# CliqueOfficial/zk-dcap-verifier

Measured on AMD Instinct MI355X. Metric: proofs/hour sgx_dcap_verifier k=19 (create_proof on the GPU: commitments, lookups, grand products, NTTs, evaluate_h, evaluations, SHPLONK, host transcript; witness synthesis excluded), higher is better.
Workload: dtype u32x8 (256-bit Montgomery integers)

## Files before the change

### zk-dcap-verifier_amd/csrc/capi.hip

```cpp
#include <string.h>
#include <new>
#include <system_error>
#include "quotient.h"

namespace zk {
int ntt_set_lds_attr();
int quotient_set_lds_attr();
int domain_lagrange_to_coeff(zk_ctx* ctx, void* d_a, uint32_t k);
int domain_coeff_to_lagrange(zk_ctx* ctx, void* d_a, uint32_t k);
int domain_lagrange_to_coeff_batch(zk_ctx* ctx, void* const* cols, size_t count, uint32_t k);
int domain_coeff_to_extended_batch(zk_ctx* ctx, const void* const* coeffs, void* const* outs, size_t count, uint32_t k, uint32_t ek);
int ntt_dev_batch(zk_ctx* ctx, void* const* h_cols, const void* const* h_srcs, size_t count, uint32_t log_n, const u256& omega, const NttFuse* fuse);
int domain_coeff_to_extended(zk_ctx* ctx, const void* d_coeff, uint32_t k, uint32_t ek, void* d_out);
int domain_extended_to_coeff(zk_ctx* ctx, void* d_a, uint32_t k, uint32_t ek);
int domain_divide_by_vanishing(zk_ctx* ctx, void* d_a, uint32_t k, uint32_t ek);
int fr_vec_op(zk_ctx* ctx, int op, const void* a, const void* b, void* out, size_t n, const u256* scalar);
int permutation_product(zk_ctx* ctx, const void* const* values, const void* const* sigmas, size_t count, uint32_t k, const void* beta, const void* gamma,
                        const void* delta_start, const void* z_init, const void* blinding, uint32_t bf, void* d_z, void* h_last_z);
int lookup_product(zk_ctx* ctx, const void* cin, const void* ctab, const void* pin, const void* ptab, uint32_t k, const void* beta, const void* gamma,
                   const void* blinding, uint32_t bf, void* d_z);
int permutation_product_circuits(zk_ctx* ctx, const void* const* values, const void* const* sigmas, size_t m, size_t n_circuits, uint32_t chunk_len, uint32_t k,
                                 const void* beta, const void* gamma, const void* blinding, uint32_t bf, void* const* d_zs);
int lookup_product_batch(zk_ctx* ctx, const void* const* cols4, size_t count, uint32_t k, const void* beta, const void* gamma, const void* blinding,
                         uint32_t bf, void* const* d_zs);
// ... 136 lines not shown
    std::unique_ptr<zk_ctx> ctx(new zk_ctx());
    ctx->device = device_id;
    if (hipStreamCreateWithFlags(&ctx->stream, hipStreamNonBlocking) != hipSuccess) return ZK_ERR_HIP;
    msm_set_lds_attr();
    ntt_set_lds_attr();
    quotient_set_lds_attr();
    *out = ctx.release();
    return ZK_OK;
} ZK_ABI_CATCH(nullptr)

}
zk_ctx* zk_internal_helper_ctx(zk_ctx* ctx) {
    if (!ctx) return nullptr;
    zk_ctx* h;
    {
        LOCK;
        h = ctx->helper;
    }
    if (!h) {
        zk_ctx* made = nullptr;
        if (zk_ctx_create(ctx->device, &made) != ZK_OK) return nullptr;
#ifndef ZK_EMU
        {
            int lane_prio;
            { LOCK; lane_prio = ctx->tune.prover_lane_priority; }
            int least = 0, greatest = 0;
            hipStream_t s = nullptr;
            if (lane_prio && hipDeviceGetStreamPriorityRange(&least, &greatest) == hipSuccess && least != greatest &&
                hipStreamCreateWithPriority(&s, hipStreamNonBlocking, lane_prio == 1 ? least : greatest) == hipSuccess) {
                (void)hipStreamDestroy(made->stream);
                made->stream = s;
            }
        }
#endif
        {
            LOCK;
            if (!ctx->helper) { ctx->helper = made; made = nullptr; }
            h = ctx->helper;
        }
        if (made) zk_ctx_destroy(made);
    }
    zk::Tune t;
    bool timing;
    {
        LOCK;
        t = ctx->tune; timing = ctx->timing;
    }
    std::lock_guard<std::mutex> lk(h->mu);
    h->tune = t;
    h->timing = timing;
    return h;
}
static void release_workspaces(zk_ctx* ctx) {
    zk::DevBuf* bufs[] = {&ctx->ws_scalars, &ctx->ws_sorted, &ctx->ws_mid, &ctx->ws_small, &ctx->ws_sub0, &ctx->ws_sub1, &ctx->ws_cls0,
                          &ctx->ws_cls1, &ctx->ws_tmp, &ctx->ws_ntt, &ctx->ws_ntt_in, &ctx->ws_pts, &ctx->ws_runs, &ctx->ws_quot, &ctx->ws_quot_state};
    for (auto* b : bufs) b->release();
}
void zk_internal_trim_helper(zk_ctx* ctx) {
    if (!ctx) return;
    zk_ctx* h;
    { LOCK; h = ctx->helper; }
    if (!h) return;
    std::lock_guard<std::mutex> lk(h->mu);
    (void)hipSetDevice(h->device);
    (void)hipStreamSynchronize(h->stream);
    release_workspaces(h);
    release_twiddles(h);
}
extern "C" {
void zk_ctx_destroy(zk_ctx* ctx) ZK_ABI_TRY {
    if (!ctx) return;
    zk_ctx* helper;
    { LOCK; helper = ctx->helper; ctx->helper = nullptr; }
    if (helper) zk_ctx_destroy(helper);
    zk_internal_plonk_ctx_destroyed(ctx);
    (void)zk_plonk_trim(ctx);
    {
        LOCK;
        (void)hipSetDevice(ctx->device);
        (void)hipStreamSynchronize(ctx->stream);
        ctx->bases.clear();
        drop_pending_timers(ctx);
        release_twiddles(ctx);
        release_pks(ctx);
        release_mock_sessions(ctx);
        release_programs(ctx);
        release_gtab(ctx);
        release_workspaces(ctx);
        (void)hipStreamDestroy(ctx->stream);
    }
    delete ctx;
} ZK_ABI_CATCH_VOID(ctx)

const char* zk_last_error(zk_ctx* ctx) ZK_ABI_TRY { return ctx ? ctx->err : "null context"; } ZK_ABI_CATCH_VALUE(ctx, "zkmi355: internal error")

static int* tune_slot(zk_ctx* ctx, const char* key) {
    zk::Tune& t = ctx->tune;
    struct { const char* k; int* v; } tab[] = {
        {"msm_c", &t.msm_c}, {"msm_sort_wgs", &t.msm_sort_wgs}, {"msm_sort_threads", &t.msm_sort_threads}, {"msm_sort_batch_wgs", &t.msm_sort_batch_wgs}, {"msm_bsort_threads", &t.msm_bsort_threads}, {"msm_bsort_chunk", &t.msm_bsort_chunk}, {"msm_wide_bins_log", &t.msm_wide_bins_log}, {"msm_part_threads", &t.msm_part_threads}, {"msm_part_pairs", &t.msm_part_pairs}, {"msm_two_level_sort", &t.msm_two_level_sort},
        {"msm_target_threads", &t.msm_target_threads}, {"msm_min_chunk", &t.msm_min_chunk}, {"msm_max_chunk", &t.msm_max_chunk},
        {"msm_max_chunk_wide", &t.msm_max_chunk_wide}, {"msm_merge_fanin", &t.msm_merge_fanin}, {"msm_tree_fanin", &t.msm_tree_fanin}, {"msm_block", &t.msm_block}, {"msm_runs", &t.msm_runs}, {"prover_side_lane", &t.prover_side_lane}, {"prover_lane_priority", &t.prover_lane_priority},
        {"ntt_tile_log", &t.ntt_tile_log}, {"ntt_threads", &t.ntt_threads}, {"ntt_max_radix_log", &t.ntt_max_radix_log}, {"ntt_plan", &t.ntt_plan}, {"ntt_full_twiddle_max_log", &t.ntt_full_twiddle_max_log}, {"ntt_coset_table", &t.ntt_coset_table}, {"ntt_col_major", &t.ntt_col_major},
        {"vec_block", &t.vec_block}, {"quot_threads", &t.quot_threads},
        {"ntt_quarter_input", &t.ntt_quarter_input}, {"ntt_fuse_scale", &t.ntt_fuse_scale}, {"quot_piece_cosets", &t.quot_piece_cosets}, {"quot_factor_horner", &t.quot_factor_horner}, {"quot_degree_split", &t.quot_degree_split}, {"quot_group_factors", &t.quot_group_factors}, {"ntt_ws_limit_mb", &t.ntt_ws_limit_mb}, 
        {"quot_jit", &t.quot_jit}, {"quot_jit_group", &t.quot_jit_group}, {"quot_jit_waves", &t.quot_jit_waves}, {"quot_remat_ops", &t.quot_remat_ops}, {"quot_remat_distance", &t.quot_remat_distance}, {"keygen_wgs", &t.keygen_wgs}, {"mock_edge_wgs", &t.mock_edge_wgs}};
    for (auto& e : tab) if (!strcmp(e.k, key)) return e.v;
    return nullptr;
// ... 330 lines not shown
```

### zk-dcap-verifier_amd/csrc/ctx.h

```cpp
#pragma once
#include <stdarg.h>
#include <string.h>
#include <stdio.h>
#include <list>
#include <map>
#include <memory>
#include <mutex>
#include <string>
#include <vector>
#include "ec.cuh"
#include "../../include/zkmi355.h"
#include "abi_guard.h"

namespace zk {

struct Tune {
    int msm_c = 0;
    int msm_sort_wgs = 256;
    int msm_sort_threads = 1024;
    int msm_bsort_threads = 1024;
    int msm_bsort_chunk = 8192;
    int msm_part_threads = 1024, msm_part_pairs = 16384;
    int msm_wide_bins_log = 9;
    int msm_two_level_sort = 0;
// ... 58 lines not shown
    void reset() { if (p) (void)hipFree(p); p = nullptr; }
};

struct TableMem {
    void* p = nullptr;
    int device = 0;
    ~TableMem() { if (p) { (void)hipSetDevice(device); (void)hipFree(p); } }
};
struct BaseTable {
    void* d_table = nullptr;
    size_t n = 0;
    int c = 0, W = 0;
    std::shared_ptr<TableMem> mem;
    void* d_runs_table = nullptr;
    std::shared_ptr<TableMem> runs_mem;
};

struct TwiddleSet {
    uint32_t log_n = 0;
    u256 omega;
    void* d_lo = nullptr;
    void* d_hi = nullptr;
    uint32_t lo_bits = 0;
    void* d_stage[3] = {nullptr, nullptr, nullptr};
    void* d_stage_sh[3] = {nullptr, nullptr, nullptr};
    void* d_stage29[3] = {nullptr, nullptr, nullptr};
    void* d_full[3] = {nullptr, nullptr, nullptr};
    uint32_t radix_log[3] = {0, 0, 0};
    int passes = 0;
    bool scale_fused = false;
    u256 fused_scale;
    uint64_t stamp = 0;
};

struct QuotProgram;
struct MockSession;

}

struct zk_ctx {
    int device = 0;
    std::mutex mu;
    char err[640] = {0};
    hipStream_t stream = nullptr;
    zk::Tune tune;
    uint64_t next_handle = 1;
    std::map<uint64_t, zk::BaseTable> bases;
    std::list<zk::TwiddleSet> twiddles;
    uint64_t twiddle_clock = 0;
    std::map<uint64_t, void*> coset_tables;
    std::map<uint64_t, std::shared_ptr<zk::QuotProgram>> programs;
    std::map<uint64_t, std::shared_ptr<zk::MockSession>> mock_sessions;
    std::map<uint64_t, std::vector<uint32_t>> lookup_tie_hint;
    zk::DevBuf ws_scalars, ws_sorted, ws_mid, ws_small, ws_sub0, ws_sub1, ws_cls0, ws_cls1, ws_tmp, ws_ntt, ws_ntt_in, ws_pts, ws_runs, ws_quot, ws_quot_state;
    bool timing = false;
    std::map<std::string, double> last_ms;
    struct PendingTimer { const char* label; hipEvent_t a, b; };
    std::vector<PendingTimer> pending_timers;
    zk_ctx* helper = nullptr;

    int fail(int code, const char* fmt, ...) {
        char buf[sizeof err];
        va_list ap;
        va_start(ap, fmt);
        vsnprintf(buf, sizeof buf, fmt, ap);
        va_end(ap);
        memcpy(err, buf, sizeof err);
        return code;
    }
};

#define ZK_HIP(call)                                                                          \
    do {                                                                                      \
        hipError_t e__ = (call);                                                              \
        if (e__ != hipSuccess)                                                                \
            return ctx->fail(ZK_ERR_HIP, "%s failed: %s (%s:%d)", #call, hipGetErrorString(e__), __FILE__, __LINE__); \
    } while (0)
#define ZK_CHECK_LAUNCH() ZK_HIP(hipGetLastError())

namespace zk {
inline void resolve_pending_timers(zk_ctx* ctx);
struct EvTimer {
    zk_ctx* ctx; const char* label; hipEvent_t a = nullptr, b = nullptr; bool on;
    EvTimer(zk_ctx* c, const char* l) : ctx(c), label(l), on(c->timing) {
        if (on) { (void)hipEventCreate(&a); (void)hipEventCreate(&b); (void)hipEventRecord(a, ctx->stream); }
    }
    void stop() { if (on) (void)hipEventRecord(b, ctx->stream); }
    void resolve() {
        if (!on) return;
        (void)hipEventSynchronize(b);
        float ms = 0; (void)hipEventElapsedTime(&ms, a, b);
        on = false;
        (void)hipEventDestroy(a); (void)hipEventDestroy(b);
        ctx->last_ms[label] += ms; ctx->last_ms[std::string(label) + "#n"] += 1.0;
    }
    void defer() {
        if (!on) return;
        if (ctx->pending_timers.size() >= 4096) resolve_pending_timers(ctx);
        ctx->pending_timers.push_back({label, a, b});
        on = false;
    }
    ~EvTimer() { if (on) { (void)hipEventDestroy(a); (void)hipEventDestroy(b); } }
    EvTimer(const EvTimer&) = delete;
    EvTimer& operator=(const EvTimer&) = delete;
};
inline void resolve_pending_timers(zk_ctx* ctx) {
    std::vector<zk_ctx::PendingTimer> list;
// ... 40 lines not shown
```

### zk-dcap-verifier_amd/csrc/msm.hip

```cpp
#include "ctx.h"
#include <algorithm>
#include <math.h>

namespace zk {

template <class F>
ZK_HD void for_each_digit(u256 s, int c, int W, F&& f) {
    const uint32_t mask = (1u << c) - 1u, half = 1u << (c - 1);
    uint32_t carry = 0;
    for (int j = 0; j < W; j++) {
        uint32_t d = (s.v[0] & mask) + carry;
#pragma unroll
        for (int i = 0; i < 7; i++) s.v[i] = (s.v[i] >> c) | (s.v[i + 1] << (32 - c));
        s.v[7] >>= c;
        if (d > half) {
            carry = 1;
            uint32_t m = (1u << c) - d;
            if (m) f(j, m, true);
        } else {
            carry = 0;
            if (d) f(j, d, false);
        }
    }
}
// ... 24 lines not shown
    uint32_t carry = 0;
#pragma unroll
    for (int j = 0; j < 16; j++) {
        const uint32_t d = ((s.v[j >> 1] >> (16 * (j & 1))) & 0xffffu) + carry;
        if (d > 0x8000u) {
            carry = 1;
            const uint32_t m = 0x10000u - d;
            if (m) f(j, m, true);
        } else {
            carry = 0;
            if (d) f(j, d, false);
        }
    }
}
template <int J = 0, class F>
ZK_HD void for_each_digit16_static(const u256& s, F&& f, uint32_t carry = 0) {
    if constexpr (J < 16) {
        const uint32_t d = ((s.v[J >> 1] >> (16 * (J & 1))) & 0xffffu) + carry;
        uint32_t cy = 0;
        if (d > 0x8000u) {
            cy = 1;
            const uint32_t m = 0x10000u - d;
            if (m) f(WinIdx<J>{}, m, true);
        } else if (d) f(WinIdx<J>{}, d, false);
        for_each_digit16_static<J + 1>(s, f, cy);
    }
}

ZK_HD uint32_t find_segment(const uint32_t* arr, uint32_t B, uint32_t j) {
    uint32_t lo = 0, hi = B;
    while (hi - lo > 1) {
        uint32_t mid = (lo + hi) >> 1;
        if (arr[mid] <= j) lo = mid; else hi = mid;
    }
    return lo;
}

ZK_HD uint32_t ceil_div(uint32_t a, uint32_t b) { return (a + b - 1) / b; }

constexpr int MSM_MAX_LEVELS = 12;
struct MsmPlan {
    uint32_t n, n_table, B, L, M, Mlog, R, nb;
    int c, W;
    const void* const* scalars;
    const void* table;
    const void* const* col_tables;
    uint32_t* small;
    uint32_t small_stride, o_off, o_cursor, o_suboff, o_info, o_tiles, o_fulloff, o_remorder, o_remhist, o_remstart, o_remcursor;
    uint32_t* sorted;
    uint64_t sorted_stride;
    uint32_t low_bits, nbin, pch, bch, o_bintot, o_bincur, o_binbase, o_chunkbase;
    uint32_t* mid_ref;
    uint16_t* mid_low;
    void* sub[2];
    uint64_t sub_stride[2];
    void* cls[2];
    uint32_t lo_bits;
};
ZK_HD uint32_t* plan_small(const MsmPlan& p, uint32_t col) { return p.small + (size_t)col * p.small_stride; }
ZK_HD const uint32_t* plan_suboff(const MsmPlan& p, uint32_t col, uint32_t level) { return plan_small(p, col) + p.o_suboff + (size_t)level * (p.B + 1); }
ZK_HD uint32_t plan_eff_levels(const MsmPlan& p, uint32_t max_s) {
    uint32_t pw = 1, r = 0;
    while (pw < max_s && r < p.R) { pw *= p.M; r++; }
    return r;
}

constexpr uint32_t MSM_MAX_BINS = 2048, MSM_MAX_LOW = 8192;
constexpr int MSM_MAX_C = 22;

__device__ __forceinline__ void block_incscan(uint32_t* v, uint32_t* tmp, uint32_t N) {
    for (uint32_t d = 1; d < N; d <<= 1) {
        for (uint32_t t = threadIdx.x; t < N; t += blockDim.x) tmp[t] = v[t] + (t >= d ? v[t - d] : 0u);
        __syncthreads();
        for (uint32_t t = threadIdx.x; t < N; t += blockDim.x) v[t] = tmp[t];
        __syncthreads();
    }
}

ZK_KERNEL void msm_bin_hist_kernel(MsmPlan p) {
    __shared__ uint32_t lh[MSM_MAX_BINS];
    const uint32_t col = blockIdx.y;
    const void* scalars = p.scalars[col];
    for (uint32_t b = threadIdx.x; b < p.nbin; b += blockDim.x) lh[b] = 0;
    __syncthreads();
    const uint32_t chunk = ceil_div(p.n, gridDim.x);
    const uint32_t lo = blockIdx.x * chunk;
    const uint32_t hi = lo + chunk < p.n ? lo + chunk : p.n;
    for (uint32_t i = lo + threadIdx.x; i < hi; i += blockDim.x) {
        u256 s = Fr::from_mont(load_u256(scalars, i));
        for_each_digit(s, p.c, p.W, [&](int, uint32_t mag, bool) { atomicAdd(&lh[(mag - 1) >> p.low_bits], 1u); });
    }
    __syncthreads();
    uint32_t* tot = plan_small(p, col) + p.o_bintot;
    for (uint32_t b = threadIdx.x; b < p.nbin; b += blockDim.x) {
        uint32_t v = lh[b];
        if (v) atomicAdd(&tot[b], v);
    }
}

ZK_KERNEL void msm_bin_base_kernel(MsmPlan p) {
    __shared__ uint32_t v[MSM_MAX_BINS], w[MSM_MAX_BINS], tmp[MSM_MAX_BINS];
    uint32_t* sm = plan_small(p, blockIdx.x);
    for (uint32_t b = threadIdx.x; b < p.nbin; b += blockDim.x) { const uint32_t t = sm[p.o_bintot + b]; v[b] = t; w[b] = ceil_div(t, p.bch); }
    __syncthreads();
    block_incscan(v, tmp, p.nbin);
    block_incscan(w, tmp, p.nbin);
    for (uint32_t b = threadIdx.x; b < p.nbin; b += blockDim.x) { sm[p.o_binbase + b + 1] = v[b]; sm[p.o_chunkbase + b + 1] = w[b]; }
    if (threadIdx.x == 0) { sm[p.o_binbase] = 0; sm[p.o_chunkbase] = 0; }
}

constexpr uint32_t PART_SPT = 2;
ZK_KERNEL void msm_partition_kernel(MsmPlan p) {
    ZK_DYN_SHARED(uint32_t, st_ref);
    const uint32_t col = blockIdx.y, nbin = p.nbin, cap = p.pch * (uint32_t)p.W;
    uint32_t* st_key = st_ref + cap;
    uint32_t* cnt = st_key + cap;
    uint32_t* start = cnt + nbin;
    uint32_t* dst = start + nbin;
// ... 338 lines not shown
}

ZK_KERNEL void ZK_LAUNCH_BOUNDS(256) ZK_WAVES_PER_EU(4) msm_accumulate_kernel(MsmPlan p) {
    const uint32_t col = blockIdx.y, B = p.B;
    const uint32_t j = blockIdx.x * blockDim.x + threadIdx.x;
    const uint32_t* sm = plan_small(p, col);
    const uint32_t* fulloff = sm + p.o_fulloff;
    const uint32_t n_full = fulloff[B];
    uint32_t b, k;
    if (j < n_full) {
        b = find_segment(fulloff, B, j);
        k = j - fulloff[b];
    } else {
        if (j - n_full >= sm[p.o_info + 1]) return;
        b = sm[p.o_remorder + (j - n_full)];
        k = fulloff[b + 1] - fulloff[b];
    }
    const uint32_t* off = sm + p.o_off;
    const uint32_t* sorted = p.sorted + (size_t)col * p.sorted_stride;
    uint32_t q = off[b] + k * p.L;
    const uint32_t bend = off[b + 1];
    const uint32_t end = q + p.L < bend ? q + p.L : bend;
    const uint32_t out = plan_suboff(p, col, 0)[b] + k;
    uint32_t ref = sorted[q];
    const void* table = p.col_tables ? p.col_tables[col] : p.table;
    Affine pt = load_affine(table, ref & 0x7fffffffu);
    XYZZ acc = xyzz_identity();
    {
        XYZZ29 a29 = xyzz29_identity();
        bool fast = !affine_is_identity(pt);
        if (fast) {
            a29.x = Fq29::enter(pt.x);
            a29.y = Fq29::enter((ref >> 31) ? Fq::neg(pt.y) : pt.y);
            a29.zz = Fq29::one(); a29.zzz = Fq29::one();
            a29.ident = false;
            ++q;
            if (q < end) { ref = sorted[q]; pt = load_affine(table, ref & 0x7fffffffu); }
        }
        while (fast && q < end) {
            const uint32_t cur_ref = ref;
            const Affine cur = pt;
            const bool more = q + 1 < end;
            if (more) ref = sorted[q + 1];
            bool fetched = false;
            fast = !affine_is_identity(cur) && xyzz29_madd_fast(a29, cur.x, (cur_ref >> 31) ? Fq::neg(cur.y) : cur.y, [&]() {
                if (more) pt = load_affine(table, ref & 0x7fffffffu);
                fetched = true;
            });
            if (fast) ++q;
            else { ref = cur_ref; if (fetched) pt = cur; }
        }
        acc = xyzz29_leave(a29);
        if (q >= end) {
            store_xyzz(p.sub[0], (size_t)col * p.sub_stride[0] + out, acc);
            return;
        }
    }
    while (true) {
        const uint32_t cur_ref = ref;
        const Affine cur = pt;
        ++q;
        if (q < end) {
            ref = sorted[q];
            pt = load_affine(table, ref & 0x7fffffffu);
        }
        xyzz_madd_signed_lazy(acc, cur, (cur_ref >> 31) != 0);
        if (q >= end) break;
    }
    xyzz_normalize(acc);
    store_xyzz(p.sub[0], (size_t)col * p.sub_stride[0] + out, acc);
}

ZK_KERNEL void msm_merge_kernel(MsmPlan p, uint32_t r, uint32_t Mpow_prev) {
    const uint32_t col = blockIdx.y, B = p.B;
    const uint32_t* sm = plan_small(p, col);
    if (Mpow_prev >= sm[p.o_info]) return;
    const uint32_t* so_in = plan_suboff(p, col, r - 1);
    const uint32_t* so_out = plan_suboff(p, col, r);
    const uint32_t t = blockIdx.x * blockDim.x + threadIdx.x;
    if (t >= so_out[B]) return;
    const uint32_t b = find_segment(so_out, B, t);
    const uint32_t k = t - so_out[b];
    const uint32_t cnt_in = so_in[b + 1] - so_in[b];
    const void* in = p.sub[(r - 1) & 1];
    const size_t ibase = (size_t)col * p.sub_stride[(r - 1) & 1] + so_in[b] + (size_t)k * p.M;
    XYZZ acc = load_xyzz(in, ibase);
    for (uint32_t m = 1; m < p.M && k * p.M + m < cnt_in; m++) xyzz_add_lazy(acc, load_xyzz(in, ibase + m));
    xyzz_normalize(acc);
    store_xyzz(p.sub[r & 1], (size_t)col * p.sub_stride[r & 1] + t, acc);
}

constexpr uint32_t RC_T = 64;
template <uint32_t SEG>
__device__ __forceinline__ XYZZ rc_wave_sum(XYZZ acc) {
    __shared__ uint4 pl[8 * RC_T];
    const uint32_t tid = threadIdx.x;
    auto put = [&](const XYZZ& v) {
        const u256* f = &v.x;
#pragma unroll
        for (int q = 0; q < 4; q++) {
            pl[(2 * q) * RC_T + tid] = make_uint4(f[q].v[0], f[q].v[1], f[q].v[2], f[q].v[3]);
            pl[(2 * q + 1) * RC_T + tid] = make_uint4(f[q].v[4], f[q].v[5], f[q].v[6], f[q].v[7]);
        }
    };
    auto get = [&](uint32_t t) {
        XYZZ v;
        u256* f = &v.x;
#pragma unroll
        for (int q = 0; q < 4; q++) {
            const uint4 l = pl[(2 * q) * RC_T + t], h = pl[(2 * q + 1) * RC_T + t];
            f[q].v[0] = l.x; f[q].v[1] = l.y; f[q].v[2] = l.z; f[q].v[3] = l.w; f[q].v[4] = h.x; f[q].v[5] = h.y; f[q].v[6] = h.z; f[q].v[7] = h.w;
        }
        return v;
    };
    put(acc);
    __syncthreads();
    for (uint32_t d = SEG >> 1; d > 0; d >>= 1) {
        const bool on = (tid & (SEG - 1)) < d;
        if (on) { xyzz_add_lazy(acc, get(tid + d)); }
        __syncthreads();
        if (on) put(acc);
        __syncthreads();
    }
    return acc;
}
template <uint32_t RC_G>
ZK_KERNEL void msm_rowcol_kernel(MsmPlan p) {
    const uint32_t col = blockIdx.y, tid = threadIdx.x, B = p.B, lane = tid & (RC_G - 1);
    const uint32_t lo_bits = p.lo_bits, n_lo = 1u << lo_bits, n_hi = (B >> lo_bits) + 1;
    const uint32_t g = blockIdx.x * (RC_T / RC_G) + tid / RC_G;
    const uint32_t r = plan_eff_levels(p, plan_small(p, col)[p.o_info]);
    const uint32_t* so = plan_suboff(p, col, r);
    const void* buf = p.sub[r & 1];
    const size_t cbase = (size_t)col * p.sub_stride[r & 1];
    XYZZ acc = xyzz_identity();
    const bool live = g < n_hi + n_lo, row = g < n_hi;
    const uint32_t fixed = row ? g : g - n_hi, count = live ? (row ? n_lo : n_hi) : 0u;
    for (uint32_t m = lane; m < count; m += RC_G) {
        const uint32_t w = row ? ((fixed << lo_bits) | m) : ((m << lo_bits) | fixed);
        if (w >= 1 && w <= B) {
            const uint32_t b = w - 1;
            if (so[b + 1] > so[b]) xyzz_add_lazy(acc, load_xyzz(buf, cbase + so[b]));
        }
    }
    acc = rc_wave_sum<RC_G>(acc);
    xyzz_normalize(acc);
    if (live && lane == 0) store_xyzz(p.cls[0], (size_t)col * (n_hi + n_lo) + g, acc);
}
ZK_KERNEL void msm_rc_class_kernel(MsmPlan p) {
    const uint32_t col = blockIdx.y, t = blockIdx.x, tid = threadIdx.x;
    const uint32_t lo_bits = p.lo_bits, n_lo = 1u << lo_bits, n_hi = (p.B >> lo_bits) + 1, hi_bits = (uint32_t)p.c - lo_bits;
    const bool rows = t < hi_bits;
    const uint32_t bit = rows ? t : t - hi_bits, count = rows ? n_hi : n_lo;
    const size_t base = (size_t)col * (n_hi + n_lo) + (rows ? 0 : n_hi);
    XYZZ acc = xyzz_identity();
    for (uint32_t m = tid; m < count; m += RC_T)
        if ((m >> bit) & 1u) xyzz_add_lazy(acc, load_xyzz(p.cls[0], base + m));
    acc = rc_wave_sum<RC_T>(acc);
    xyzz_normalize(acc);
    if (tid == 0) store_xyzz(p.cls[1], (size_t)col * p.c + t, acc);
}

ZK_KERNEL void g1_affine_to_xyzz_kernel(const void* aff, uint32_t n, void* out) {
    const uint32_t i = blockIdx.x * blockDim.x + threadIdx.x;
    if (i >= n) return;
    store_xyzz(out, i, xyzz_from_affine(load_affine(aff, i)));
}
ZK_KERNEL void g1_dbl_times_kernel(void* pts, uint32_t n, int times) {
    const uint32_t i = blockIdx.x * blockDim.x + threadIdx.x;
    if (i >= n) return;
    XYZZ p = load_xyzz(pts, i);
    for (int k = 0; k < times; k++) p = xyzz_dbl(p);
    store_xyzz(pts, i, p);
}
ZK_KERNEL void g1_batch_to_affine_kernel(const void* in, uint32_t n, uint32_t chunk, void* out) {
    const uint32_t t = blockIdx.x * blockDim.x + threadIdx.x;
    const uint64_t lo64 = (uint64_t)t * chunk;
    if (lo64 >= n) return;
    const uint32_t lo = (uint32_t)lo64;
    const uint32_t hi = lo + chunk < n ? lo + chunk : n;
    u256 acc = Fq::one();
    for (uint32_t k = lo; k < hi; k++) {
        u256 zz = load_u256(in, 4 * (size_t)k + 2), zzz = load_u256(in, 4 * (size_t)k + 3);
        store_u256(out, 2 * (size_t)k, acc);
        if (!Fq::is_zero(zz)) acc = Fq::mul(acc, Fq::mul(zz, zzz));
    }
    u256 inv = Fq::inv(acc);
// ... 192 lines not shown
    int rc = build_table(ctx, d_aff, n, ps);
    if (rc) return rc;
    bt.d_runs_table = ps.d_table;
    bt.runs_mem = ps.mem;
    return ZK_OK;
}

int msm_release(zk_ctx* ctx, uint64_t handle) {
    auto it = ctx->bases.find(handle);
    if (it == ctx->bases.end()) return ctx->fail(ZK_ERR_ARG, "zk_bases_release: unknown handle %llu", (unsigned long long)handle);
    ctx->bases.erase(it);
    return ZK_OK;
}

static void xyzz_to_jacobian_host(const XYZZ& p, void* out96) {
    u256* o = reinterpret_cast<u256*>(out96);
    if (xyzz_is_identity(p)) { o[0] = Fq::zero(); o[1] = Fq::zero(); o[2] = Fq::zero(); return; }
    u256 I = Fq::inv(Fq::mul(p.zz, p.zzz));
    o[0] = Fq::mul(p.x, Fq::mul(I, p.zzz));
    o[1] = Fq::mul(p.y, Fq::mul(I, p.zz));
    o[2] = Fq::one();
}
static void xyzz_batch_to_jacobian_host(const std::vector<XYZZ>& pts, void* out) {
    const size_t nb = pts.size();
    std::vector<u256> pre(nb);
    u256 acc = Fq::one();
    for (size_t i = 0; i < nb; i++) { pre[i] = acc; if (!xyzz_is_identity(pts[i])) acc = Fq::mul(acc, Fq::mul(pts[i].zz, pts[i].zzz)); }
    u256 inv = Fq::inv(acc);
    for (size_t i = nb; i-- > 0;) {
        u256* o = reinterpret_cast<u256*>((char*)out + i * 96);
        const XYZZ& p = pts[i];
        if (xyzz_is_identity(p)) { o[0] = Fq::zero(); o[1] = Fq::zero(); o[2] = Fq::zero(); continue; }
        u256 I = Fq::mul(inv, pre[i]);
        inv = Fq::mul(inv, Fq::mul(p.zz, p.zzz));
        o[0] = Fq::mul(p.x, Fq::mul(I, p.zzz));
        o[1] = Fq::mul(p.y, Fq::mul(I, p.zz));
        o[2] = Fq::one();
    }
}

static int msm_core(zk_ctx* ctx, const BaseTable& bt, const void* const* h_scal_ptrs, uint32_t nb, size_t n, XYZZ* out_xyzz, const void* const* h_col_tables = nullptr) {
    const int c = bt.c, W = bt.W;
    const uint32_t B = 1u << (c - 1);
    const Tune& tn = ctx->tune;
    const uint64_t pairs_max = (uint64_t)n * W;
    uint32_t Mlog = 1;
    while ((2u << Mlog) <= (uint32_t)std::max(2, tn.msm_merge_fanin) && Mlog < 8) Mlog++;
    const uint32_t M = 1u << Mlog;
    uint32_t L = (uint32_t)std::min<uint64_t>(std::max<uint64_t>((uint64_t)nb * pairs_max / (uint64_t)tn.msm_target_threads, (uint64_t)tn.msm_min_chunk),
                                              (uint64_t)(c > 16 ? tn.msm_max_chunk_wide : tn.msm_max_chunk));
    MsmPlan p;
    memset(&p, 0, sizeof p);
    p.n = (uint32_t)n; p.n_table = (uint32_t)bt.n; p.B = B; p.L = L; p.M = M; p.Mlog = Mlog; p.nb = nb; p.c = c; p.W = W;
    uint64_t cap[MSM_MAX_LEVELS + 1];
    cap[0] = pairs_max / L + B + 1;
    uint32_t R = 0;
    {
        uint64_t worst = pairs_max / L + 1;
        while (worst > 1 && R < MSM_MAX_LEVELS) { worst = (worst + M - 1) / M; R++; cap[R] = cap[R - 1] / M + B + 1; }
        if (worst > 1) return ctx->fail(ZK_ERR_LIMIT, "zk_msm: merge depth exceeds %d levels (raise msm_merge_fanin)", MSM_MAX_LEVELS);
    }
    p.R = R;
    p.o_off = B; p.o_cursor = p.o_off + B + 1; p.o_suboff = p.o_cursor + B; p.o_info = p.o_suboff + (R + 1) * (B + 1);
    const uint32_t scan_tiles = ceil_div(B, SC_TILE);
    p.o_tiles = p.o_info + 4;
    p.o_fulloff = p.o_tiles + scan_tiles * SC_NV;
    p.o_remorder = p.o_fulloff + B + 1;
    p.o_remhist = p.o_remorder + B;
    p.o_remstart = p.o_remhist + REM_CLASSES;
    p.o_remcursor = p.o_remstart + REM_CLASSES;
    p.o_bintot = p.o_remcursor + REM_CLASSES;
    p.low_bits = c <= 16 ? (uint32_t)std::min(7, c - 1) : (uint32_t)std::max(c - 1 - std::min(std::max(tn.msm_wide_bins_log, 8), 11), 5);
    p.nbin = B >> p.low_bits;
    p.bch = (uint32_t)std::max(64, tn.msm_bsort_chunk);
    p.o_bincur = p.o_bintot + p.nbin;
    p.o_binbase = p.o_bincur + p.nbin;
    p.o_chunkbase = p.o_binbase + p.nbin + 1;
    p.small_stride = p.o_chunkbase + p.nbin + 1;
    const int part_threads = std::min(std::max(tn.msm_part_threads, 64), std::min(1024, tn.msm_sort_threads));
    p.pch = std::min<uint32_t>(std::max<uint32_t>(1, (uint32_t)std::min(std::max(tn.msm_part_pairs, 64), 16384) / (uint32_t)W), PART_SPT * (uint32_t)part_threads);
    if (p.nbin > MSM_MAX_BINS || (1u << p.low_bits) > MSM_MAX_LOW) return ctx->fail(ZK_ERR_LIMIT, "zk_msm: window width c = %d exceeds %d", c, MSM_MAX_C);
    ZK_HIP(ctx->ws_small.ensure((size_t)nb * p.small_stride * 4 + 2 * (size_t)nb * sizeof(void*) + 64));
    p.small = (uint32_t*)ctx->ws_small.p;
    const void** d_ptrs = (const void**)((char*)ctx->ws_small.p + (((size_t)nb * p.small_stride * 4 + 15) & ~(size_t)15));
    p.scalars = d_ptrs;
    p.table = bt.d_table;
    p.col_tables = h_col_tables ? d_ptrs + nb : nullptr;
    p.sorted_stride = (pairs_max + 4 + 15) & ~(uint64_t)15;
    ZK_HIP(ctx->ws_sorted.ensure((size_t)nb * p.sorted_stride * 4));
    p.sorted = (uint32_t*)ctx->ws_sorted.p;
    ZK_HIP(ctx->ws_mid.ensure((size_t)nb * p.sorted_stride * 6 + 64));
    p.mid_ref = (uint32_t*)ctx->ws_mid.p;
    p.mid_low = (uint16_t*)((char*)ctx->ws_mid.p + (size_t)nb * p.sorted_stride * 4);
    p.sub_stride[0] = cap[0];
    p.sub_stride[1] = R >= 1 ? cap[1] : 1;
    ZK_HIP(ctx->ws_sub0.ensure((size_t)nb * p.sub_stride[0] * 128));
    ZK_HIP(ctx->ws_sub1.ensure((size_t)nb * p.sub_stride[1] * 128));
    p.sub[0] = ctx->ws_sub0.p; p.sub[1] = ctx->ws_sub1.p;
    p.lo_bits = (uint32_t)(c - 1 + 1) / 2;
    const uint32_t n_groups = (B >> p.lo_bits) + 1 + (1u << p.lo_bits);
    ZK_HIP(ctx->ws_cls0.ensure((size_t)nb * n_groups * 128));
    ZK_HIP(ctx->ws_cls1.ensure((size_t)nb * c * 128 + 128));
    p.cls[0] = ctx->ws_cls0.p; p.cls[1] = ctx->ws_cls1.p;

    hipStream_t st = ctx->stream;
    ZK_HIP(hipMemsetAsync(p.small, 0, (size_t)nb * p.small_stride * 4, st));
    ZK_HIP(hipMemcpyAsync((void*)d_ptrs, h_scal_ptrs, (size_t)nb * sizeof(void*), hipMemcpyHostToDevice, st));
    if (h_col_tables) ZK_HIP(hipMemcpyAsync((void*)(d_ptrs + nb), h_col_tables, (size_t)nb * sizeof(void*), hipMemcpyHostToDevice, st));
    int wgs = tn.msm_sort_wgs;
    {
        uint64_t per = (uint64_t)tn.msm_sort_threads * 4;
        uint64_t want = (n + per - 1) / per;
        if (want < (uint64_t)wgs) wgs = (int)std::max<uint64_t>(want, 1);
        if (nb > 1) wgs = std::max(1, std::min(wgs, (int)((tn.msm_sort_batch_wgs) / nb) + 1));
    }
    const uint64_t chunk_max = std::min<uint64_t>((uint64_t)SC_SPT * tn.msm_sort_threads, 65536 / (uint64_t)W);
    const uint64_t need = (n + chunk_max - 1) / chunk_max;
    const bool two_level = W > (int)SC_WMAX || c > 16 || tn.msm_two_level_sort != 0;
    const uint32_t bsort_grid = (uint32_t)(pairs_max / p.bch) + p.nbin;
    EvTimer t_sort(ctx, "msm_sort");
    if (two_level) {
        ZK_LAUNCH(msm_bin_hist_kernel, dim3(wgs, nb), tn.msm_sort_threads, 0, st, p);
        ZK_CHECK_LAUNCH();
        ZK_LAUNCH(msm_bin_base_kernel, nb, 256, 0, st, p);
        ZK_CHECK_LAUNCH();
        ZK_LAUNCH(msm_partition_kernel, dim3(ceil_div(p.n, p.pch), nb), part_threads, ((size_t)p.pch * W * 2 + 4 * (size_t)p.nbin) * 4, st, p);
        ZK_CHECK_LAUNCH();
        ZK_LAUNCH(msm_bsort_count_kernel, dim3(bsort_grid, nb), tn.msm_bsort_threads, (size_t)4 << p.low_bits, st, p);
        ZK_CHECK_LAUNCH();
    } else {
        ZK_LAUNCH(msm_hist_kernel, dim3(wgs, nb), tn.msm_sort_threads, (size_t)B * 4, st, p);
        ZK_CHECK_LAUNCH();
    }
    ZK_LAUNCH(msm_scan_tiles_kernel, dim3(scan_tiles, nb), SC_T, 0, st, p);
    ZK_CHECK_LAUNCH();
    ZK_LAUNCH(msm_scan_tilesums_kernel, nb, 64, 0, st, p, scan_tiles);
    ZK_CHECK_LAUNCH();
    ZK_LAUNCH(msm_scan_apply_kernel, dim3(scan_tiles, nb), SC_T, 0, st, p);
    ZK_CHECK_LAUNCH();
    if (two_level) {
        ZK_LAUNCH(msm_bsort_place_kernel, dim3(bsort_grid, nb), tn.msm_bsort_threads, (size_t)4 << p.low_bits, st, p);
        ZK_CHECK_LAUNCH();
    } else {
        ZK_LAUNCH(msm_scatter_kernel, dim3((uint32_t)std::max<uint64_t>(need, (uint64_t)wgs), nb), tn.msm_sort_threads, (size_t)B * 4, st, p);
        ZK_CHECK_LAUNCH();
    }
    t_sort.stop();

    const int blk = tn.msm_block;
    EvTimer t_acc(ctx, "msm_accumulate");
    if (blk > 256) return ctx->fail(ZK_ERR_ARG, "msm_block: at most 256 threads per workgroup");
    {
        const dim3 grid((uint32_t)((cap[0] + blk - 1) / blk), nb);
        ZK_LAUNCH(msm_accumulate_kernel, grid, blk, 0, st, p);
    }
    ZK_CHECK_LAUNCH();
    t_acc.stop();

    EvTimer t_red(ctx, "msm_reduce");
    {
        uint64_t pw = 1;
        for (uint32_t r = 1; r <= R; r++) {
            ZK_LAUNCH(msm_merge_kernel, dim3((uint32_t)((cap[r] + blk - 1) / blk), nb), blk, 0, st, p, r, (uint32_t)std::min<uint64_t>(pw, 0xffffffffull));
            ZK_CHECK_LAUNCH();
            pw *= M;
        }
    }
    if (nb >= 4) { ZK_LAUNCH(msm_rowcol_kernel<16>, dim3((n_groups + 3) / 4, nb), RC_T, 0, st, p); }
    else { ZK_LAUNCH(msm_rowcol_kernel<64>, dim3(n_groups, nb), RC_T, 0, st, p); }
    ZK_CHECK_LAUNCH();
    ZK_LAUNCH(msm_rc_class_kernel, dim3((uint32_t)c, nb), RC_T, 0, st, p);
    ZK_CHECK_LAUNCH();
    t_red.stop();
    std::vector<XYZZ> cls((size_t)nb * c);
    ZK_HIP(hipMemcpyAsync(cls.data(), p.cls[1], (size_t)nb * c * 128, hipMemcpyDeviceToHost, st));
    std::vector<uint32_t> npairs(ctx->timing ? nb : 0);
    for (uint32_t col = 0; col < (uint32_t)npairs.size(); col++)
        ZK_HIP(hipMemcpyAsync(&npairs[col], plan_small(p, col) + p.o_off + B, 4, hipMemcpyDeviceToHost, st));
    ZK_HIP(hipStreamSynchronize(st));
    for (uint32_t v : npairs) ctx->last_ms["msm_pairs"] += (double)v;
    if (ctx->timing) ctx->last_ms["msm_columns"] += (double)nb;
    t_sort.resolve(); t_acc.resolve(); t_red.resolve();
    const int hi_bits = c - (int)p.lo_bits;
    for (uint32_t col = 0; col < nb; col++) {
        const XYZZ* cc = &cls[(size_t)col * c];
        XYZZ h = cc[hi_bits - 1];
        for (int t = hi_bits - 2; t >= 0; t--) { h = xyzz_dbl(h); xyzz_add(h, cc[t]); }
        for (uint32_t t = 0; t < p.lo_bits; t++) h = xyzz_dbl(h);
        XYZZ l = cc[c - 1];
        for (int t = (int)p.lo_bits - 2; t >= 0; t--) { l = xyzz_dbl(l); xyzz_add(l, cc[hi_bits + t]); }
        xyzz_add(h, l);
        out_xyzz[col] = h;
    }
    return ZK_OK;
}

int msm_run_batch(zk_ctx* ctx, uint64_t handle, const void* const* scalars, size_t nb, size_t n, bool on_device, void* out, int partial) {
    auto it = ctx->bases.find(handle);
    if (it == ctx->bases.end()) return ctx->fail(ZK_ERR_ARG, "zk_msm: unknown bases handle %llu", (unsigned long long)handle);
    const BaseTable& bt = it->second;
    if (nb == 0) return ZK_OK;
    if (!out || !scalars) return ctx->fail(ZK_ERR_ARG, "zk_msm: null pointer");
    if (n > bt.n) return ctx->fail(ZK_ERR_ARG, "zk_msm: n = %zu exceeds registered table size %zu", n, bt.n);
    if (nb > 4096) return ctx->fail(ZK_ERR_LIMIT, "zk_msm_batch: more than 4096 columns");
    std::vector<XYZZ> res(nb, xyzz_identity());
    if (n > 0) {
        std::vector<const void*> ptrs(nb);
        for (size_t i = 0; i < nb; i++) {
            if (!scalars[i]) return ctx->fail(ZK_ERR_ARG, "zk_msm: null scalar column %zu", i);
            ptrs[i] = scalars[i];
        }
        if (!on_device) {
            ZK_HIP(ctx->ws_scalars.ensure(nb * n * 32));
            for (size_t i = 0; i < nb; i++) {
                void* d = (char*)ctx->ws_scalars.p + i * n * 32;
                ZK_HIP(hipMemcpyAsync(d, scalars[i], n * 32, hipMemcpyHostToDevice, ctx->stream));
                ptrs[i] = d;
            }
        }
        std::vector<uint32_t> direct, runs;
// ... 118 lines not shown
```

Before: 70550.

## Replace multi-level MSM merge launches with one in-place per-bucket tree merge

The per-level MSM merge kernels, which ping-pong between two sub-sum buffers, are replaced by a single kernel. Each workgroup owns 256 buckets and reduces their partial sums in place with a strided M-ary tree, synchronising between levels. This drops the second workspace buffer, the per-level launches and the level bookkeeping, and the row/column stage now reads level-0 offsets directly. The costs are strided, less coalesced loads at the higher levels, and serialised work inside one workgroup when a few buckets hold many partial sums.

```diff
diff --git a/zk-dcap-verifier_amd/csrc/capi.hip b/zk-dcap-verifier_amd/csrc/capi.hip
--- a/zk-dcap-verifier_amd/csrc/capi.hip
+++ b/zk-dcap-verifier_amd/csrc/capi.hip
@@ -212,7 +212,7 @@
     return h;
 }
 static void release_workspaces(zk_ctx* ctx) {
-    zk::DevBuf* bufs[] = {&ctx->ws_scalars, &ctx->ws_sorted, &ctx->ws_mid, &ctx->ws_small, &ctx->ws_sub0, &ctx->ws_sub1, &ctx->ws_cls0,
+    zk::DevBuf* bufs[] = {&ctx->ws_scalars, &ctx->ws_sorted, &ctx->ws_mid, &ctx->ws_small, &ctx->ws_sub0, &ctx->ws_cls0,
                           &ctx->ws_cls1, &ctx->ws_tmp, &ctx->ws_ntt, &ctx->ws_ntt_in, &ctx->ws_pts, &ctx->ws_runs, &ctx->ws_quot, &ctx->ws_quot_state};
     for (auto* b : bufs) b->release();
 }
diff --git a/zk-dcap-verifier_amd/csrc/ctx.h b/zk-dcap-verifier_amd/csrc/ctx.h
--- a/zk-dcap-verifier_amd/csrc/ctx.h
+++ b/zk-dcap-verifier_amd/csrc/ctx.h
@@ -134,7 +134,7 @@
     std::map<uint64_t, std::shared_ptr<zk::QuotProgram>> programs;
     std::map<uint64_t, std::shared_ptr<zk::MockSession>> mock_sessions;
     std::map<uint64_t, std::vector<uint32_t>> lookup_tie_hint;
-    zk::DevBuf ws_scalars, ws_sorted, ws_mid, ws_small, ws_sub0, ws_sub1, ws_cls0, ws_cls1, ws_tmp, ws_ntt, ws_ntt_in, ws_pts, ws_runs, ws_quot, ws_quot_state;
+    zk::DevBuf ws_scalars, ws_sorted, ws_mid, ws_small, ws_sub0, ws_cls0, ws_cls1, ws_tmp, ws_ntt, ws_ntt_in, ws_pts, ws_runs, ws_quot, ws_quot_state;
     bool timing = false;
     std::map<std::string, double> last_ms;
     struct PendingTimer { const char* label; hipEvent_t a, b; };
diff --git a/zk-dcap-verifier_amd/csrc/msm.hip b/zk-dcap-verifier_amd/csrc/msm.hip
--- a/zk-dcap-verifier_amd/csrc/msm.hip
+++ b/zk-dcap-verifier_amd/csrc/msm.hip
@@ -100,18 +100,13 @@
     uint32_t low_bits, nbin, pch, bch, o_bintot, o_bincur, o_binbase, o_chunkbase;
     uint32_t* mid_ref;
     uint16_t* mid_low;
-    void* sub[2];
-    uint64_t sub_stride[2];
+    void* sub;
+    uint64_t sub_stride;
     void* cls[2];
     uint32_t lo_bits;
 };
 ZK_HD uint32_t* plan_small(const MsmPlan& p, uint32_t col) { return p.small + (size_t)col * p.small_stride; }
 ZK_HD const uint32_t* plan_suboff(const MsmPlan& p, uint32_t col, uint32_t level) { return plan_small(p, col) + p.o_suboff + (size_t)level * (p.B + 1); }
-ZK_HD uint32_t plan_eff_levels(const MsmPlan& p, uint32_t max_s) {
-    uint32_t pw = 1, r = 0;
-    while (pw < max_s && r < p.R) { pw *= p.M; r++; }
-    return r;
-}
 
 constexpr uint32_t MSM_MAX_BINS = 2048, MSM_MAX_LOW = 8192;
 constexpr int MSM_MAX_C = 22;
@@ -556,7 +551,7 @@
         }
         acc = xyzz29_leave(a29);
         if (q >= end) {
-            store_xyzz(p.sub[0], (size_t)col * p.sub_stride[0] + out, acc);
+            store_xyzz(p.sub, (size_t)col * p.sub_stride + out, acc);
             return;
         }
     }
@@ -572,26 +567,43 @@
         if (q >= end) break;
     }
     xyzz_normalize(acc);
-    store_xyzz(p.sub[0], (size_t)col * p.sub_stride[0] + out, acc);
-}
-
-ZK_KERNEL void msm_merge_kernel(MsmPlan p, uint32_t r, uint32_t Mpow_prev) {
-    const uint32_t col = blockIdx.y, B = p.B;
-    const uint32_t* sm = plan_small(p, col);
-    if (Mpow_prev >= sm[p.o_info]) return;
-    const uint32_t* so_in = plan_suboff(p, col, r - 1);
-    const uint32_t* so_out = plan_suboff(p, col, r);
-    const uint32_t t = blockIdx.x * blockDim.x + threadIdx.x;
-    if (t >= so_out[B]) return;
-    const uint32_t b = find_segment(so_out, B, t);
-    const uint32_t k = t - so_out[b];
-    const uint32_t cnt_in = so_in[b + 1] - so_in[b];
-    const void* in = p.sub[(r - 1) & 1];
-    const size_t ibase = (size_t)col * p.sub_stride[(r - 1) & 1] + so_in[b] + (size_t)k * p.M;
-    XYZZ acc = load_xyzz(in, ibase);
-    for (uint32_t m = 1; m < p.M && k * p.M + m < cnt_in; m++) xyzz_add_lazy(acc, load_xyzz(in, ibase + m));
-    xyzz_normalize(acc);
-    store_xyzz(p.sub[r & 1], (size_t)col * p.sub_stride[r & 1] + t, acc);
+    store_xyzz(p.sub, (size_t)col * p.sub_stride + out, acc);
+}
+
+constexpr uint32_t MG_T = 256;
+ZK_KERNEL void ZK_LAUNCH_BOUNDS(MG_T) msm_merge_kernel(MsmPlan p) {
+    __shared__ uint32_t cnt[MG_T], ends[MG_T], tmp[MG_T];
+    const uint32_t col = blockIdx.y, tid = threadIdx.x, M = p.M;
+    const uint32_t b0 = blockIdx.x * MG_T;
+    const uint32_t nbk = p.B - b0 < MG_T ? p.B - b0 : MG_T;
+    const uint32_t* so = plan_suboff(p, col, 0) + b0;
+    const size_t cbase = (size_t)col * p.sub_stride;
+    cnt[tid] = tid < nbk ? so[tid + 1] - so[tid] : 0u;
+    __syncthreads();
+    for (size_t stride = 1;; stride *= M) {
+        ends[tid] = cnt[tid] > 1 ? ceil_div(cnt[tid], M) : 0u;
+        __syncthreads();
+        block_incscan(ends, tmp, MG_T);
+        const uint32_t total = ends[MG_T - 1];
+        if (total == 0) break;
+        for (uint32_t t = tid; t < total; t += MG_T) {
+            uint32_t lo = 0, hi = MG_T - 1;
+            while (lo < hi) {
+                const uint32_t mid = (lo + hi) >> 1;
+                if (ends[mid] > t) hi = mid; else lo = mid + 1;
+            }
+            const uint32_t first = (t - (lo ? ends[lo - 1] : 0u)) * M, c = cnt[lo];
+            if (first + 1 >= c) continue;
+            const size_t base = cbase + so[lo] + first * stride;
+            XYZZ acc = load_xyzz(p.sub, base);
+            for (uint32_t m = 1; m < M && first + m < c; m++) xyzz_add_lazy(acc, load_xyzz(p.sub, base + m * stride));
+            xyzz_normalize(acc);
+            store_xyzz(p.sub, base, acc);
+        }
+        __syncthreads();
+        if (cnt[tid] > 1) cnt[tid] = ceil_div(cnt[tid], M);
+        __syncthreads();
+    }
 }
 
 constexpr uint32_t RC_T = 64;
@@ -633,10 +645,9 @@
     const uint32_t col = blockIdx.y, tid = threadIdx.x, B = p.B, lane = tid & (RC_G - 1);
     const uint32_t lo_bits = p.lo_bits, n_lo = 1u << lo_bits, n_hi = (B >> lo_bits) + 1;
     const uint32_t g = blockIdx.x * (RC_T / RC_G) + tid / RC_G;
-    const uint32_t r = plan_eff_levels(p, plan_small(p, col)[p.o_info]);
-    const uint32_t* so = plan_suboff(p, col, r);
-    const void* buf = p.sub[r & 1];
-    const size_t cbase = (size_t)col * p.sub_stride[r & 1];
+    const uint32_t* so = plan_suboff(p, col, 0);
+    const void* buf = p.sub;
+    const size_t cbase = (size_t)col * p.sub_stride;
     XYZZ acc = xyzz_identity();
     const bool live = g < n_hi + n_lo, row = g < n_hi;
     const uint32_t fixed = row ? g : g - n_hi, count = live ? (row ? n_lo : n_hi) : 0u;
@@ -935,14 +946,8 @@
     MsmPlan p;
     memset(&p, 0, sizeof p);
     p.n = (uint32_t)n; p.n_table = (uint32_t)bt.n; p.B = B; p.L = L; p.M = M; p.Mlog = Mlog; p.nb = nb; p.c = c; p.W = W;
-    uint64_t cap[MSM_MAX_LEVELS + 1];
-    cap[0] = pairs_max / L + B + 1;
-    uint32_t R = 0;
-    {
-        uint64_t worst = pairs_max / L + 1;
-        while (worst > 1 && R < MSM_MAX_LEVELS) { worst = (worst + M - 1) / M; R++; cap[R] = cap[R - 1] / M + B + 1; }
-        if (worst > 1) return ctx->fail(ZK_ERR_LIMIT, "zk_msm: merge depth exceeds %d levels (raise msm_merge_fanin)", MSM_MAX_LEVELS);
-    }
+    const uint64_t cap0 = pairs_max / L + B + 1;
+    const uint32_t R = 0;
     p.R = R;
     p.o_off = B; p.o_cursor = p.o_off + B + 1; p.o_suboff = p.o_cursor + B; p.o_info = p.o_suboff + (R + 1) * (B + 1);
     const uint32_t scan_tiles = ceil_div(B, SC_TILE);
@@ -975,11 +980,9 @@
     ZK_HIP(ctx->ws_mid.ensure((size_t)nb * p.sorted_stride * 6 + 64));
     p.mid_ref = (uint32_t*)ctx->ws_mid.p;
     p.mid_low = (uint16_t*)((char*)ctx->ws_mid.p + (size_t)nb * p.sorted_stride * 4);
-    p.sub_stride[0] = cap[0];
-    p.sub_stride[1] = R >= 1 ? cap[1] : 1;
-    ZK_HIP(ctx->ws_sub0.ensure((size_t)nb * p.sub_stride[0] * 128));
-    ZK_HIP(ctx->ws_sub1.ensure((size_t)nb * p.sub_stride[1] * 128));
-    p.sub[0] = ctx->ws_sub0.p; p.sub[1] = ctx->ws_sub1.p;
+    p.sub_stride = cap0;
+    ZK_HIP(ctx->ws_sub0.ensure((size_t)nb * p.sub_stride * 128));
+    p.sub = ctx->ws_sub0.p;
     p.lo_bits = (uint32_t)(c - 1 + 1) / 2;
     const uint32_t n_groups = (B >> p.lo_bits) + 1 + (1u << p.lo_bits);
     ZK_HIP(ctx->ws_cls0.ensure((size_t)nb * n_groups * 128));
@@ -1034,21 +1037,15 @@
     EvTimer t_acc(ctx, "msm_accumulate");
     if (blk > 256) return ctx->fail(ZK_ERR_ARG, "msm_block: at most 256 threads per workgroup");
     {
-        const dim3 grid((uint32_t)((cap[0] + blk - 1) / blk), nb);
+        const dim3 grid((uint32_t)((cap0 + blk - 1) / blk), nb);
         ZK_LAUNCH(msm_accumulate_kernel, grid, blk, 0, st, p);
     }
     ZK_CHECK_LAUNCH();
     t_acc.stop();
 
     EvTimer t_red(ctx, "msm_reduce");
-    {
-        uint64_t pw = 1;
-        for (uint32_t r = 1; r <= R; r++) {
-            ZK_LAUNCH(msm_merge_kernel, dim3((uint32_t)((cap[r] + blk - 1) / blk), nb), blk, 0, st, p, r, (uint32_t)std::min<uint64_t>(pw, 0xffffffffull));
-            ZK_CHECK_LAUNCH();
-            pw *= M;
-        }
-    }
+    ZK_LAUNCH(msm_merge_kernel, dim3(ceil_div(B, MG_T), nb), MG_T, 0, st, p);
+    ZK_CHECK_LAUNCH();
     if (nb >= 4) { ZK_LAUNCH(msm_rowcol_kernel<16>, dim3((n_groups + 3) / 4, nb), RC_T, 0, st, p); }
     else { ZK_LAUNCH(msm_rowcol_kernel<64>, dim3(n_groups, nb), RC_T, 0, st, p); }
     ZK_CHECK_LAUNCH();
```

Result: no change. 70480, median of 2 (-0.1%).
